# manuelinfosec/corrosion

Hardware: AMD Instinct MI355X
Metric: merged column-changes/sec (node) at 1/2/4/8 GPUs + % of HBM BW roofline (higher is better)
Workload: dtype int64; 1 GPU; config 2: 64M column-changes, 1 table x 4 INTEGER cols, 1000 actors, uniform pk in [1,2^22], cl=1, one apply into an empty state per step; changes=67108864, cells=16469597, parallelism=1 GPU

## Files before the change

corrosion_amd/csrc/engine.hip:

```cpp
#include <hip/hip_runtime.h>

#include <algorithm>
#include <chrono>
#include <cstdlib>
#include <cstring>
#include <mutex>
#include <numeric>

#include "internal.h"
#include "merge_kernels.h"

namespace corro {

static thread_local std::string g_last_error;

void set_error(const std::string &msg) { g_last_error = msg; }

int fail(int code, const std::string &msg) {
    g_last_error = msg;
    return code;
}

int DevBuf::ensure(size_t want) {
    if (want <= bytes && p) return CORRO_OK;
// ... 391 lines not shown
int corro_abi_version(void) { return CORRO_HIP_ABI_VERSION; }

int corro_device_count(int *count) {
    if (!count) return fail(CORRO_E_INVALID, "count is NULL");
    int c = 0;
    hipError_t e = hipGetDeviceCount(&c);
    if (e != hipSuccess) c = 0;
    *count = c;
    return CORRO_OK;
}

static int ctx_prepare_device(corro_ctx *ctx) {
    int c = 0;
    if (hipGetDeviceCount(&c) != hipSuccess || c == 0)
        return fail(CORRO_E_NO_DEVICE, "no HIP device visible: the merge engine has no CPU fallback");
    if (ctx->device < 0 || ctx->device >= c) return fail(CORRO_E_INVALID, "device ordinal out of range");
    CORRO_HIP_TRY(hipSetDevice(ctx->device));
    hipDeviceProp_t prop;
    CORRO_HIP_TRY(hipGetDeviceProperties(&prop, ctx->device));
    if (std::strncmp(prop.gcnArchName, "gfx950", 6) != 0)
        return fail(CORRO_E_NO_DEVICE, std::string("libcorro_hip is built for gfx950, device is ") + prop.gcnArchName);
    CORRO_HIP_TRY(hipStreamCreateWithFlags(&ctx->stream, hipStreamNonBlocking));
    CORRO_HIP_TRY(hipHostMalloc((void **)&ctx->h_misc, MISC_WORDS * sizeof(uint64_t), hipHostMallocDefault));
    for (auto &e : ctx->ev) CORRO_HIP_TRY(hipEventCreate(&e));
    const size_t lds_max = 160 * 1024;
    for (const void *f : {(const void *)k_hist<8>, (const void *)k_hist<16>, (const void *)k_hist<32>,
                          (const void *)k_hist<16, true>, (const void *)k_hist<16, false, true>})
        CORRO_HIP_TRY(hipFuncSetAttribute(f, hipFuncAttributeMaxDynamicSharedMemorySize, (int)lds_max));
    for (const void *f : {(const void *)k_scatter<true, true>, (const void *)k_scatter<true, false>,
                          (const void *)k_scatter<true, false, 8>,
                          (const void *)k_scatter<false, true>, (const void *)k_scatter<false, false>})
        CORRO_HIP_TRY(hipFuncSetAttribute(f, hipFuncAttributeMaxDynamicSharedMemorySize, (int)lds_max));
    return CORRO_OK;
}

}

static int store_alloc(corro_ctx *ctx, uint64_t capacity_hint) {
    const uint32_t B = ctx->B;
    const uint64_t rows = std::max<uint64_t>(1024, capacity_hint / 16);
    uint32_t lg = 4;
    while (((uint64_t)B << lg) < 2 * rows && lg < 20 && ((uint64_t)B << (lg + 1)) <= (1ULL << 31)) lg++;
    ctx->log2S = lg;
    TRY(ctx->d_ent.ensure(((size_t)B << lg) * sizeof(RowEnt)));
    TRY(ctx->d_used.ensure(B * 4ULL));
    TRY(ctx->d_gen.ensure(B * 4ULL));
    TRY(ctx->d_heap_top.ensure(8));
    ctx->heap_cap = std::min<uint64_t>(1ULL << 31, std::max<uint64_t>(1ULL << 16, capacity_hint / 2));
    TRY(ctx->d_heap.ensure(ctx->heap_cap * sizeof(Rec)));
    return CORRO_OK;
}

static int store_clear(corro_ctx *ctx) {
    hipStream_t s = ctx->stream;
    CORRO_HIP_TRY(hipMemsetAsync(ctx->d_ent.p, 0, ((size_t)ctx->B << ctx->log2S) * sizeof(RowEnt), s));
    CORRO_HIP_TRY(hipMemsetAsync(ctx->d_used.p, 0, ctx->B * 4ULL, s));
    CORRO_HIP_TRY(hipMemsetAsync(ctx->d_gen.p, 0, ctx->B * 4ULL, s));
    CORRO_HIP_TRY(hipMemsetAsync(ctx->d_heap_top.p, 0, 8, s));
    if (ctx->d_touch_n.p) CORRO_HIP_TRY(hipMemsetAsync(ctx->d_touch_n.p, 0, 8, s));
    ctx->touch_bound = 0;
    ctx->state_total = 0;
    ctx->state_rows = 0;
    ctx->arena_top = 0;
    ctx->vc_last_bytes = 0;
    ctx->state_epoch++;
    ctx->poisoned = false;
    return CORRO_OK;
}

namespace corro {
RowStore row_store(corro_ctx *ctx) {
    RowStore rs{};
    rs.ent = ctx->d_ent.as<RowEnt>();
    rs.used = ctx->d_used.as<uint32_t>();
    rs.gen = ctx->d_gen.as<uint32_t>();
    rs.heap = ctx->d_heap.as<Rec>();
    rs.heap_ts = ctx->track_ts ? ctx->d_heap_ts.as<uint64_t>() : nullptr;
    rs.heap_top = ctx->d_heap_top.as<unsigned long long>();
    rs.heap_cap = ctx->heap_cap;
    rs.log2S = ctx->log2S;
    rs.fill = (uint32_t)((7ULL << ctx->log2S) >> 3);
    rs.stride = ctx->d_stride.as<uint16_t>();
// ... 98 lines not shown
        }
        Table tb;
        tb.name = tables[t].name;
        for (uint32_t c = 0; c < tables[t].ncols; c++) tb.cols.emplace_back(tables[t].col_names[c]);
        ctx->max_stride = std::max<uint32_t>(ctx->max_stride, tables[t].ncols + 1);
        ctx->table_index[tb.name] = t;
        ctx->tables.push_back(std::move(tb));
    }
    uint64_t per = std::max<uint64_t>(1, capacity_hint / 1280);
    uint32_t lg = 0;
    while ((1ULL << lg) < per && lg < 15) lg++;
    ctx->log2B = lg;
    ctx->B = 1u << lg;
    int rc = ctx_prepare_device(ctx);
    if (rc != CORRO_OK) {
        corro_ctx_destroy(ctx);
        return rc;
    }
    const uint32_t B = ctx->B;
    rc = ctx->d_new_cnt.ensure(B * 4ULL);
    if (!rc) rc = ctx->d_stage_off.ensure(B * 4ULL);
    if (!rc) rc = ctx->d_bflags.ensure(((B + 31) / 32) * 4ULL);
    if (!rc) rc = ctx->d_misc.ensure(MISC_WORDS * 8);
    if (!rc) rc = ctx->d_ovf_list.ensure(B * 4ULL);
    if (!rc) rc = ctx->d_gen_list.ensure(3 * B * 4ULL);
    if (!rc) rc = ctx->d_wide_list.ensure(B * 4ULL);
    if (!rc) rc = ctx->d_defer.ensure(B * 4ULL);
    if (!rc) rc = ctx->d_relist.ensure(B * 4ULL);
    if (!rc) rc = store_alloc(ctx, capacity_hint);
    if (rc != CORRO_OK) {
        corro_ctx_destroy(ctx);
        return rc;
    }
    {
        std::vector<uint16_t> ncols(ctx->tables.size() + 1, 0), stride(ctx->tables.size() + 1, 1);
        for (size_t t = 0; t < ctx->tables.size(); t++) {
            ncols[t] = (uint16_t)ctx->tables[t].cols.size();
            stride[t] = (uint16_t)(ctx->tables[t].cols.size() + 1);
        }
        rc = ctx->d_ncols.ensure(ncols.size() * 2);
        if (!rc) rc = ctx->d_stride.ensure(stride.size() * 2);
        if (rc == CORRO_OK &&
            (hipMemcpy(ctx->d_ncols.p, ncols.data(), ncols.size() * 2, hipMemcpyHostToDevice) != hipSuccess ||
             hipMemcpy(ctx->d_stride.p, stride.data(), stride.size() * 2, hipMemcpyHostToDevice) != hipSuccess))
            rc = fail(CORRO_E_DEVICE, "upload of the schema failed");
        if (rc == CORRO_OK) rc = store_clear(ctx);
        if (rc == CORRO_OK) rc = prims_warm(ctx);
        if (rc == CORRO_OK) rc = agent_dev_reserve(ctx, std::max<uint64_t>(4096, capacity_hint / 64));
        if (rc != CORRO_OK) {
            corro_ctx_destroy(ctx);
            return rc;
        }
    }
    *out = ctx;
    return CORRO_OK;
}

void corro_ctx_destroy(corro_ctx *ctx) {
    if (!ctx) return;
    if (ctx->stream) (void)hipStreamSynchronize(ctx->stream);
    DevBuf *bufs[] = {&ctx->d_site_rank, &ctx->d_dbv, &ctx->d_dbv_batch, &ctx->d_ent, &ctx->d_used, &ctx->d_gen,
                      &ctx->d_heap, &ctx->d_heap_ts, &ctx->d_heap_top, &ctx->d_stride, &ctx->d_defer,
                      &ctx->d_relist, &ctx->d_dense, &ctx->d_dense_ts, &ctx->d_dense_view, &ctx->d_in,
                      &ctx->d_hist, &ctx->d_new_cnt, &ctx->d_stage_off, &ctx->d_bflags, &ctx->d_stage,
                      &ctx->d_misc, &ctx->d_ovf_list, &ctx->d_gen_list, &ctx->d_wide_list, &ctx->d_fast_of, &ctx->d_ovf_sort, &ctx->d_ovf_rcl, &ctx->d_ovf_sum, &ctx->d_ovf_plan, &ctx->d_setdbv,
                      &ctx->d_scan_tmp, &ctx->d_impact, &ctx->d_export, &ctx->d_needs, &ctx->d_needs1,
                      &ctx->d_xidx, &ctx->d_xout, &ctx->d_wire, &ctx->d_wire_schema, &ctx->d_wire_sites,
                      &ctx->d_ncols, &ctx->d_part, &ctx->d_arena, &ctx->d_aff, &ctx->d_affflag,
                      &ctx->d_agent_in, &ctx->d_agent_batch, &ctx->d_agent_spans, &ctx->d_agent_imp,
                      &ctx->d_agent_out, &ctx->d_agent_aux, &ctx->d_agent_fetch, &ctx->d_agent_aux2, &ctx->d_touch, &ctx->d_touch_n, &ctx->d_touch_stamp, &ctx->d_touch_tmp,
                      &ctx->d_aff_conv, &ctx->d_aff_vals, &ctx->d_gaps_big, &ctx->d_agent_hdr, &ctx->d_wire_map,
                      &ctx->d_hdr_stage, &ctx->d_pm_ts};
    for (DevBuf *b : bufs) b->release();
    ctx->d_pkdir.release();
    ctx->d_pk_scratch.release();
    ctx->d_pk_bad.release();
    ctx->d_part_var.release();
    for (PkTable &t : ctx->pk) {
        t.d_off.release();
        t.d_bytes.release();
        t.d_hash.release();
        t.d_slots.release();
    }
    if (ctx->h_misc) (void)hipHostFree(ctx->h_misc);
    if (ctx->h_ovf) (void)hipHostFree(ctx->h_ovf);
    if (ctx->h_agent) (void)hipHostFree(ctx->h_agent);
    if (ctx->h_hdr) (void)hipHostFree(ctx->h_hdr);
    if (ctx->h_hfetch) (void)hipHostFree(ctx->h_hfetch);
// ... 141 lines not shown
static int apply_chunk(corro_ctx *ctx, BatchDev bd, uint8_t *imp_buf) {
    hipStream_t s = ctx->stream;
    const uint32_t n = bd.n;
    const uint32_t B = ctx->B, log2B = ctx->log2B;
    const uint32_t nsites = (uint32_t)ctx->sites.size();
    if (bd.ts && !ctx->track_ts) {
        TRY(ctx->d_heap_ts.ensure(ctx->heap_cap * 8));
        CORRO_HIP_TRY(hipMemsetAsync(ctx->d_heap_ts.p, 0, ctx->heap_cap * 8, s));
        ctx->track_ts = true;
    }

    static const uint32_t tiles_max = [] {
        const char *e = std::getenv("CORRO_HIP_TILES");
        const long v = e ? std::atol(e) : 0;
        return v > 0 && v <= 4096 ? (uint32_t)v : TILES_MAX;
    }();
    uint32_t ntiles = std::max<uint32_t>(1, std::min<uint32_t>(tiles_max, (n + 4095) / 4096));
    uint32_t tile = (n + ntiles - 1) / ntiles;
    tile = (tile + HIST_THREADS - 1) / HIST_THREADS * HIST_THREADS;
    ntiles = (n + tile - 1) / tile;

    TRY(ctx->d_hist.ensure((size_t)ntiles * B * 4));
    TRY(ctx->d_stage.ensure((size_t)n * sizeof(Rec)));
    ApplyZero z{ctx->d_bflags.as<uint32_t>(), ctx->d_misc.as<unsigned long long>(),
                ctx->d_dbv_batch.as<unsigned long long>(), (B + 31) / 32, (uint32_t)MISC_WORDS, nsites};
    if (imp_buf) CORRO_HIP_TRY(hipMemsetAsync(imp_buf, 0, bd.ap ? ctx->pm_n : n, s));

    unsigned long long *misc = ctx->d_misc.as<unsigned long long>();
    const bool prof = ctx->profiling;
    auto mark = [&](int i) {
        if (prof) (void)hipEventRecord(ctx->ev[i], s);
    };
    for (int k = 0; k < 6; k++) ctx->last_ms[k] = 0.f;
    mark(0);
    const uint32_t one_table = ctx->tables.size() == 1 ? 1u : 0u;
    static const int hist_u = std::getenv("CORRO_HIST_U") ? std::atoi(std::getenv("CORRO_HIST_U")) : 16;
    using HistK = void (*)(BatchDev, uint32_t, uint32_t, uint32_t, uint32_t *, ApplyZero);
    const HistK hk = bd.slot_rec ? k_hist<16, true>
                     : !one_table ? (HistK)k_hist<16, false, true>
                     : hist_u == 8 ? k_hist<8> : hist_u == 32 ? k_hist<32> : k_hist<16>;
    hipLaunchKernelGGL(hk, dim3(ntiles), dim3(HIST_THREADS), (size_t)B * 4, s, bd, tile, log2B, one_table,
                       ctx->d_hist.as<uint32_t>(), z);
    CORRO_HIP_TRY(hipGetLastError());
    mark(1);
    hipLaunchKernelGGL(k_colscan, dim3((B + 255) / 256), dim3(256), 0, s, ctx->d_hist.as<uint32_t>(), ntiles, B,
                       ctx->d_new_cnt.as<uint32_t>());
    mark(2);
    hipLaunchKernelGGL(k_plan, dim3(1), dim3(1024), 0, s, ctx->d_new_cnt.as<uint32_t>(), B,
                       ctx->d_stage_off.as<uint32_t>());
    mark(3);
    {
        static const bool nt_stores = std::getenv("CORRO_HIP_NT") && std::atoi(std::getenv("CORRO_HIP_NT")) != 0;
        const bool plain = !bd.v1 && !bd.vt && !bd.vl && !bd.conv;
        if (bd.ts_v1 && !plain) return fail(CORRO_E_INVALID, "internal: ts_v1 on a batch with value words");
        static const bool scat8 = std::getenv("CORRO_SCAT_U") && std::atoi(std::getenv("CORRO_SCAT_U")) == 8;
        auto kern = plain ? (nt_stores ? k_scatter<true, true> : scat8 ? k_scatter<true, false, 8> : k_scatter<true, false>)
                          : (nt_stores ? k_scatter<false, true> : k_scatter<false, false>);
        hipLaunchKernelGGL(kern, dim3(ntiles), dim3(HIST_THREADS), (size_t)B * 4 + ((B + 31) / 32) * 4, s, bd,
                           tile, log2B, one_table, ctx->d_hist.as<uint32_t>(), ctx->d_stage_off.as<uint32_t>(),
                           ctx->d_stage.as<Rec>(), ctx->d_bflags.as<uint32_t>(),
                           ctx->d_dbv_batch.as<unsigned long long>(), nsites, ctx->d_ncols.as<uint16_t>(),
                           (uint32_t)ctx->tables.size(), misc);
    }
    CORRO_HIP_TRY(hipGetLastError());
    mark(4);

    MergeArgs a{};
    a.stage = ctx->d_stage.as<Rec>();
    a.stage_off = ctx->d_stage_off.as<uint32_t>();
    a.new_cnt = ctx->d_new_cnt.as<uint32_t>();
    a.bflags = ctx->d_bflags.as<uint32_t>();
    a.batch_ts = bd.ts;
    a.rs = row_store(ctx);
    a.site_rank = ctx->d_site_rank.as<uint32_t>();
    a.nsites = nsites;
    a.impact = imp_buf;
    a.misc = misc;
    a.ovf_list = ctx->d_ovf_list.as<uint32_t>();
    a.gen_list = ctx->d_gen_list.as<uint32_t>();
    a.wide_list = ctx->d_wide_list.as<uint32_t>();
    a.defer_list = ctx->d_defer.as<uint32_t>();
    a.bucket_list = nullptr;
    a.B = B;
    static const bool force_general = std::getenv("CORRO_HIP_FORCE_GENERAL") &&
                                      std::atoi(std::getenv("CORRO_HIP_FORCE_GENERAL")) != 0;
    a.force_general = force_general ? 1u : 0u;
    static const char *gom = std::getenv("CORRO_GEN_OVF_MIN");
    a.gen_ovf_min = gom ? (uint32_t)std::atoi(gom)
                        : (ovf_reduce_ok(ctx, imp_buf != nullptr) && bd.n >= (1ULL << 24) ? 512u : 0xFFFFFFFFu);
    a.track_ts = ctx->track_ts ? 1u : 0u;
    a.state_wide = ctx->state_wide ? 1u : 0u;
    a.arena = ctx->d_arena.as<uint8_t>();
    a.touch = ctx->track_touched ? ctx->d_touch.as<uint4>() : nullptr;
    a.touch_n = ctx->track_touched ? ctx->d_touch_n.as<unsigned long long>() : nullptr;
    if (bd.conv) {
        a.raw = bd;
        a.raw.arena = ctx->d_arena.as<uint8_t>();
    }
    a.pos_src = bd.ap ? ctx->pm_src : nullptr;
    a.ts_v1 = bd.ts_v1;
    uint32_t nblocks = B;
    float merge_ms = 0.f, ovf_ms = 0.f;
    if (a.impact) {
        CORRO_HIP_TRY(hipMemcpyAsync(ctx->h_misc, misc, (MISC_CVBIG + 1) * 8, hipMemcpyDeviceToHost, s));
        CORRO_HIP_TRY(hipStreamSynchronize(s));
        if (ctx->h_misc[0]) return error_from_bits(ctx->h_misc[0]);
    }
    bool extra_rounds = false;
    for (int round = 0;; round++) {
        if (round > 40) return fail(CORRO_E_NOMEM, "internal: the row store did not take the batch's rows");
        mark(4);
        static const bool no_triage = std::getenv("CORRO_TRIAGE") && std::atoi(std::getenv("CORRO_TRIAGE")) == 0;
        if (!no_triage) {
            TRY(ctx->d_fast_of.ensure(B + 256));
            a.fast_of = ctx->d_fast_of.as<uint8_t>();
            hipLaunchKernelGGL(k_triage, dim3(std::min<uint32_t>((nblocks + 255) / 256, 1024)), dim3(256), 0, s, a, nblocks,
                               ctx->d_fast_of.as<uint8_t>());
            CORRO_HIP_TRY(hipGetLastError());
        }
        if (a.impact) {
            const bool packed = ctx->h_misc[MISC_CVBIG] == 0 && nsites <= 65536;
            auto kern = packed ? k_merge_fast_int<true, true> : k_merge_fast_int<true, false>;
            hipLaunchKernelGGL(kern, dim3(nblocks), dim3(FAST_T), 0, s, a);
            CORRO_HIP_TRY(hipGetLastError());
            hipLaunchKernelGGL(k_merge_fast_wide<true>, dim3(std::min(nblocks, LIST_GRID)), dim3(FAST_T), 0, s, a);
        } else {
            hipLaunchKernelGGL(k_merge_fast_int<false>, dim3(nblocks), dim3(FAST_T), 0, s, a);
            CORRO_HIP_TRY(hipGetLastError());
            hipLaunchKernelGGL(k_merge_fast_wide<false>, dim3(std::min(nblocks, LIST_GRID)), dim3(FAST_T), 0, s, a);
        }
        CORRO_HIP_TRY(hipGetLastError());
        hipLaunchKernelGGL(k_merge_gen_small, dim3(std::min(nblocks, 4 * LIST_GRID)), dim3(GEN_SMALL_THREADS), 0, s, a);
        CORRO_HIP_TRY(hipGetLastError());
        hipLaunchKernelGGL(k_merge_gen_mid, dim3(std::min(nblocks, 2 * LIST_GRID)), dim3(MERGE_THREADS), 0, s, a);
        CORRO_HIP_TRY(hipGetLastError());
        hipLaunchKernelGGL(k_merge_gen, dim3(std::min(nblocks, LIST_GRID)), dim3(MERGE_THREADS), 0, s, a);
        CORRO_HIP_TRY(hipGetLastError());
        mark(5);
        if (round == 0) {
            hipLaunchKernelGGL(k_dbv_fold, dim3((nsites + 255) / 256), dim3(256), 0, s,
                               ctx->d_dbv.as<unsigned long long>(), ctx->d_dbv_batch.as<unsigned long long>(), nsites,
                               (const unsigned long long *)misc);
            CORRO_HIP_TRY(hipMemsetAsync(misc + MISC_ROWS, 0, 8, s));
            hipLaunchKernelGGL(k_sum_used, dim3(1), dim3(1024), 0, s, ctx->d_used.as<uint32_t>(), B, misc);
        }
        CORRO_HIP_TRY(hipMemcpyAsync(ctx->h_misc, misc, MISC_WORDS * 8, hipMemcpyDeviceToHost, s));
        CORRO_HIP_TRY(hipStreamSynchronize(s));
        if (round == 0) {
            if (ctx->h_misc[0]) return error_from_bits(ctx->h_misc[0]);
            ctx->apply_wrote = true;
            if (prof)
                for (int i = 0; i < 4; i++) CORRO_HIP_TRY(hipEventElapsedTime(&ctx->last_ms[i], ctx->ev[i], ctx->ev[i + 1]));
        }
        if (prof) {
            float ms = 0.f;
            CORRO_HIP_TRY(hipEventElapsedTime(&ms, ctx->ev[4], ctx->ev[5]));
            merge_ms += ms;
        }
        const uint64_t novf = ctx->h_misc[MISC_OVF];
        if (novf) {
            extra_rounds = true;
            TRY(run_overflow(ctx, a, novf, n, prof));
            ctx->metrics.overflow_rounds++;
            ovf_ms += ctx->last_ms[5];
        }
        const uint64_t ndefer = ctx->h_misc[MISC_DEFER];
        if (!ndefer) break;
        extra_rounds = true;
        const uint64_t why = ctx->h_misc[MISC_DEFER_WHY];
        ctx->metrics.deferred_rounds++;
        if (why & DEFER_REGION) TRY(grow_regions(ctx, ctx->log2S + 1));
        if (why & DEFER_HEAP) {
            unsigned long long top = 0;
            CORRO_HIP_TRY(hipMemcpy(&top, ctx->d_heap_top.p, 8, hipMemcpyDeviceToHost));
            TRY(grow_heap(ctx, std::max<uint64_t>(ctx->heap_cap * 2, top + (top >> 2))));
        }
        CORRO_HIP_TRY(hipMemcpyAsync(ctx->d_relist.p, ctx->d_defer.p, ndefer * 4, hipMemcpyDeviceToDevice, s));
        for (int w : {MISC_OVF, MISC_GEN, MISC_WIDEQ, MISC_GEN_SMALL, MISC_GEN_MID, MISC_DEFER, MISC_DEFER_WHY})
            CORRO_HIP_TRY(hipMemsetAsync(misc + w, 0, 8, s));
        a.rs = row_store(ctx);
        a.bucket_list = ctx->d_relist.as<uint32_t>();
        nblocks = (uint32_t)ndefer;
    }
    if (prof) {
        ctx->last_ms[4] = merge_ms;
        ctx->last_ms[5] = ovf_ms;
    }
    if (extra_rounds) {
        CORRO_HIP_TRY(hipMemsetAsync(misc + MISC_ROWS, 0, 8, s));
        hipLaunchKernelGGL(k_sum_used, dim3(1), dim3(1024), 0, s, ctx->d_used.as<uint32_t>(), B, misc);
        CORRO_HIP_TRY(hipMemcpyAsync(ctx->h_misc, misc, MISC_WORDS * 8, hipMemcpyDeviceToHost, s));
        CORRO_HIP_TRY(hipStreamSynchronize(s));
    }
    ctx->state_total += ctx->h_misc[MISC_LIVE];
    ctx->state_rows = ctx->h_misc[MISC_ROWS];
#if CORRO_DIAG & 256
    fprintf(stderr, "DIAG impact phases (us per bucket; packed body: loads claims rows counts place walk region winners): %.3f %.3f %.3f %.3f %.3f %.3f %.3f %.3f\n",
            ctx->h_misc[MISC_DIAG] / 100.0 / B, ctx->h_misc[MISC_DIAG + 1] / 100.0 / B,
            ctx->h_misc[MISC_DIAG + 2] / 100.0 / B, ctx->h_misc[MISC_DIAG + 3] / 100.0 / B,
            ctx->h_misc[MISC_DIAG + 4] / 100.0 / B, ctx->h_misc[MISC_DIAG + 5] / 100.0 / B,
            ctx->h_misc[MISC_DIAG + 6] / 100.0 / B, ctx->h_misc[MISC_DIAG + 7] / 100.0 / B);
#endif
#if CORRO_DIAG & 64
    fprintf(stderr, "DIAG phases (us per bucket): load %.3f claims %.3f rows_count %.3f stage1 %.3f stages %.3f fast_rows %.3f winners %.3f publish %.3f\n",
            ctx->h_misc[MISC_DIAG] / 100.0 / B, ctx->h_misc[MISC_DIAG + 1] / 100.0 / B,
            ctx->h_misc[MISC_DIAG + 6] / 100.0 / B, ctx->h_misc[MISC_DIAG + 7] / 100.0 / B,
            ctx->h_misc[MISC_DIAG + 2] / 100.0 / B, ctx->h_misc[MISC_DIAG + 3] / 100.0 / B,
            ctx->h_misc[MISC_DIAG + 4] / 100.0 / B, ctx->h_misc[MISC_DIAG + 5] / 100.0 / B);
#endif
    ctx->state_epoch++;
    if (ctx->h_misc[MISC_WIDE]) ctx->state_wide = true;
    const uint64_t slots = (uint64_t)B << ctx->log2S;
    if (ctx->state_rows * 8 > slots * 5) {
        uint32_t lg = ctx->log2S;
// ... 573 lines not shown
```

corrosion_amd/csrc/internal.h:

```cpp
#pragma once
#include <hip/hip_runtime.h>

#include <array>
#include <cstdint>
#include <cstdlib>
#include <map>
#include <string>
#include <unordered_map>
#include <vector>

#include "corro_hip.h"

namespace corro {

inline bool fault_armed(const char *name) {
    const char *e = std::getenv("CORRO_FAULT");
    if (!e || !*e) return false;
    const std::string s = std::string(",") + e + ",";
    return s.find(std::string(",") + name + ",") != std::string::npos;
}

void set_error(const std::string &msg);
int fail(int code, const std::string &msg);

// ... 131 lines not shown
    const uint64_t *pm_ts = nullptr;
    uint64_t pm_n = 0;
    bool pm_slack = false;
    const void *slot_rec = nullptr;
    const uint64_t *slot_cnt = nullptr;
    uint32_t slot_cap = 0, slot_nsrc = 0;
    uint32_t *slot_over = nullptr;
    bool apply_wrote = false;
    uint64_t heap_limit = 0;
    bool state_wide = false;
    corro::DevBuf d_defer, d_relist;
    corro::DevBuf d_dense, d_dense_ts, d_dense_view;
    corro::DevBuf d_arena;
    uint64_t arena_top = 0;
    uint64_t vc_min_bytes = 0;
    uint64_t vc_last_bytes = 0;
    uint64_t dense_epoch = ~0ULL;

    corro::DevBuf d_in;
    corro::DevBuf d_hist;
    corro::DevBuf d_new_cnt, d_stage_off, d_bflags;
    corro::DevBuf d_stage;
    corro::DevBuf d_misc;
    corro::DevBuf d_ovf_list;
    corro::DevBuf d_gen_list;
    corro::DevBuf d_wide_list;
    corro::DevBuf d_fast_of;
    corro::DevBuf d_ovf_sort;
    corro::DevBuf d_ovf_rcl;
    corro::DevBuf d_ovf_sum;
    bool ovf_sum_dirty = false;
    corro::DevBuf d_ovf_plan;
    uint64_t ovf_temp_k = 0;
    size_t ovf_temp = 0;
    corro::DevBuf d_setdbv;
    corro::DevBuf d_scan_tmp;
    corro::DevBuf d_impact;
    corro::DevBuf d_pm_ts;
    corro::DevBuf d_export;
    corro::DevBuf d_needs;
    corro::DevBuf d_needs1;
    corro::DevBuf d_xidx;
    corro::DevBuf d_xout;
    corro::XIdxPtrs x;
    uint64_t state_epoch = 0;
    uint64_t xidx_epoch = ~0ULL;
// ... 18 lines not shown
    int aff_policy = CORRO_AFF_POLICY_SQLITE_3_37_2;
    corro::DevBuf d_part;
    corro::DevBuf d_pkdir;
    corro::DevBuf d_pk_scratch;
    corro::DevBuf d_pk_bad;
    corro::DevBuf d_part_var;
    corro::DevBuf d_agent_in, d_agent_batch, d_agent_spans, d_agent_imp, d_agent_out, d_agent_aux;
    corro::DevBuf d_agent_fetch, d_agent_aux2;
    corro::DevBuf d_agent_hdr;
    bool agent_sorted_mode = false;
    const uint32_t *agent_src_of = nullptr;
    void *h_agent = nullptr;
    size_t h_agent_bytes = 0;
    void *h_hdr = nullptr;
    size_t h_hdr_bytes = 0;
    void *h_hfetch = nullptr;
    size_t h_hfetch_bytes = 0;
    void *h_pool = nullptr;
    size_t h_pool_bytes = 0;
    corro::DevBuf d_hdr_stage;
    uint64_t agent_ncs = 0;
    uint64_t agent_nbatch_max = 0;
    uint64_t *h_misc = nullptr;
    uint32_t *h_ovf = nullptr;
    bool profiling = false;
    hipEvent_t ev[8] = {};
    float last_ms[9] = {};
};
```

corrosion_amd/csrc/merge_kernels.h:

```cpp
#pragma once
#include "internal.h"
#include "rowhash.h"
#include "rowstore.h"

namespace corro {

#ifndef CORRO_DIAG
#define CORRO_DIAG 0
#endif
constexpr int HIST_THREADS = 512;
constexpr uint64_t CV_PACKED_LIMIT = 1ULL << 15;
constexpr uint32_t TILES_MAX = 256;
constexpr int MERGE_THREADS = 512;
#ifndef CORRO_FAST_T
#define CORRO_FAST_T 512
#endif
constexpr int FAST_T = CORRO_FAST_T;
constexpr int CAP_FAST = 3072;
constexpr int FAST_R = CAP_FAST / FAST_T;
static_assert(FAST_R * FAST_T == CAP_FAST, "FAST_T must divide CAP_FAST");
constexpr int FAST_WAVES_EU = 2 * (FAST_T / 64) / 4;
constexpr int FAST_SLOTS = 4096;
#ifndef IMPACT_LISTS
#define IMPACT_LISTS 0
// ... 112 lines not shown
    w1 = ((in.lbase + off) << 24) | sz;
    return true;
}

__device__ inline void touch_append(const MergeArgs &a, uint64_t pk, uint32_t table) {
    const unsigned long long act = __ballot(1);
    const uint32_t lane = threadIdx.x & 63;
    const uint32_t leader = (uint32_t)__ffsll(act) - 1;
    const uint32_t rank = (uint32_t)__popcll(act & ((1ULL << lane) - 1ULL));
    unsigned long long base = 0;
    if (lane == leader) base = atomicAdd(a.touch_n, (unsigned long long)__popcll(act));
    base = __shfl(base, leader);
    a.touch[base + rank] = make_uint4((uint32_t)pk, (uint32_t)(pk >> 32), table, 0u);
}

__device__ inline uint32_t site_rank_of(const MergeArgs &a, uint32_t site) {
    return site < a.nsites ? a.site_rank[site] : 0u;
}

struct ApplyZero {
    uint32_t *bflags;
    unsigned long long *misc, *dbv_batch;
    uint32_t nbflags, nmisc, nsites;
};
template <int HIST_U, bool SLOT = false, bool MT = false>
static __global__ void __launch_bounds__(HIST_THREADS)
k_hist(BatchDev in, uint32_t tile, uint32_t log2B, uint32_t one_table, uint32_t *__restrict__ hist_out, ApplyZero z) {
    extern __shared__ uint32_t hist[];
    const uint32_t B = 1u << log2B;
    {
        const uint32_t t = blockIdx.x * blockDim.x + threadIdx.x, nt = gridDim.x * blockDim.x;
        for (uint32_t i = t; i < z.nbflags; i += nt) z.bflags[i] = 0;
        for (uint32_t i = t; i < z.nmisc; i += nt) z.misc[i] = 0;
        for (uint32_t i = t; i < z.nsites; i += nt) z.dbv_batch[i] = 0;
    }
    for (uint32_t i = threadIdx.x; i < B; i += blockDim.x) hist[i] = 0;
    bool sover = false;
    if constexpr (SLOT) {
        sover = slot_overflowed(in);
        if (in.slot_over && blockIdx.x == 0 && threadIdx.x == 0) *in.slot_over = sover ? 1u : 0u;
    }
    __syncthreads();
    const uint32_t begin = blockIdx.x * tile;
    const uint32_t end = min(in.n, begin + tile);
    for (uint32_t base = begin; base < end; base += blockDim.x * HIST_U) {
        uint64_t pk[HIST_U];
        uint32_t tc[HIST_U], ap[HIST_U];
#pragma unroll
        for (int k = 0; k < HIST_U; k++) {
            const uint32_t i = min(base + k * blockDim.x + threadIdx.x, end - 1);
            if constexpr (SLOT) {
                pk[k] = in.slot_rec[i].pk;
                tc[k] = one_table ? 0u : in.slot_rec[i].tcid;
                ap[k] = slot_valid(in, i, sover) ? 0u : AP_SKIP;
            } else {
                pk[k] = in.pk[i];
                tc[k] = MT ? in.tcid[i] : 0u;
                ap[k] = in.ap && !in.ap_all ? in.ap[i] : 0u;
            }
        }
#pragma unroll
        for (int k = 0; k < HIST_U; k++) {
            const uint32_t i = base + k * blockDim.x + threadIdx.x;
            if (i < end && ap[k] != AP_SKIP) atomicAdd(&hist[bucket_of(tc[k] >> 16, pk[k], log2B)], 1u);
        }
    }
    __syncthreads();
    uint32_t *row = hist_out + (size_t)blockIdx.x * B;
    for (uint32_t b = threadIdx.x; b < B; b += blockDim.x) row[b] = hist[b];
}

static __global__ void k_colscan(uint32_t *__restrict__ hist, uint32_t ntiles, uint32_t B,
                          uint32_t *__restrict__ new_cnt) {
    const uint32_t b = blockIdx.x * blockDim.x + threadIdx.x;
    if (b >= B) return;
    uint32_t run = 0;
    uint32_t t = 0;
    for (; t + 4 <= ntiles; t += 4) {
        uint32_t c[4];
#pragma unroll
        for (int k = 0; k < 4; k++) c[k] = hist[(size_t)(t + k) * B + b];
#pragma unroll
        for (int k = 0; k < 4; k++) {
            hist[(size_t)(t + k) * B + b] = run;
            run += c[k];
        }
    }
    for (; t < ntiles; t++) {
        const size_t k = (size_t)t * B + b;
        const uint32_t c = hist[k];
        hist[k] = run;
        run += c;
    }
    new_cnt[b] = run;
}

constexpr uint32_t PLAN_PER = 32;
static __global__ void __launch_bounds__(1024)
k_plan(const uint32_t *__restrict__ new_cnt, uint32_t B, uint32_t *__restrict__ stage_off) {
    __shared__ uint64_t w_a[16];
    const uint32_t lane = threadIdx.x & 63, w = threadIdx.x >> 6;
    const uint32_t per = B >= 1024 ? B / 1024 : 1u;
    const uint32_t b0 = threadIdx.x * per;
    const uint32_t cnt = b0 < B ? per : 0u;
    uint64_t sa = 0;
    if (per >= 4) {
        uint4 x[PLAN_PER / 4];
#pragma unroll
        for (uint32_t k = 0; k < PLAN_PER / 4; k++) x[k] = reinterpret_cast<const uint4 *>(new_cnt + b0)[min(k, per / 4 - 1)];
#pragma unroll
        for (uint32_t k = 0; k < PLAN_PER / 4; k++)
            if (4 * k < per) sa += (uint64_t)x[k].x + x[k].y + x[k].z + x[k].w;
    } else {
        for (uint32_t k = 0; k < cnt; k++) sa += new_cnt[b0 + k];
    }
    uint64_t ia = sa;
#pragma unroll
    for (int d = 1; d < 64; d <<= 1) {
        const uint64_t xa = __shfl_up(ia, d);
        if (lane >= (uint32_t)d) ia += xa;
    }
    if (lane == 63) w_a[w] = ia;
    __syncthreads();
    uint64_t ra = ia - sa;
    for (uint32_t ww = 0; ww < w; ww++) ra += w_a[ww];
    if (per >= 4) {
#pragma unroll
        for (uint32_t k = 0; k < PLAN_PER / 4; k++) {
            if (4 * k >= per) break;
            const uint4 xk = reinterpret_cast<const uint4 *>(new_cnt + b0)[k];
            const uint32_t xs[4] = {xk.x, xk.y, xk.z, xk.w};
            uint32_t so[4];
#pragma unroll
            for (int e = 0; e < 4; e++) {
                so[e] = (uint32_t)ra;
                ra += xs[e];
            }
            reinterpret_cast<uint4 *>(stage_off + b0)[k] = make_uint4(so[0], so[1], so[2], so[3]);
        }
    } else {
        for (uint32_t k = 0; k < cnt; k++) {
            stage_off[b0 + k] = (uint32_t)ra;
            ra += new_cnt[b0 + k];
        }
    }
}

__device__ inline void store_rec(Rec *dst, const Rec &r) {
    const uint4 *s = reinterpret_cast<const uint4 *>(&r);
    uint4 *d = reinterpret_cast<uint4 *>(dst);
    d[0] = s[0];
    d[1] = s[1];
    d[2] = s[2];
    d[3] = s[3];
}

__device__ inline Rec load_rec(const Rec *src) {
    Rec r;
    const uint4 *s = reinterpret_cast<const uint4 *>(src);
    uint4 *d = reinterpret_cast<uint4 *>(&r);
    d[0] = s[0];
    d[1] = s[1];
    d[2] = s[2];
    d[3] = s[3];
    return r;
}

__device__ inline void swap32(uint32_t &a, uint32_t &b) {
    auto r = __builtin_amdgcn_permlane32_swap(a, b, false, false);
// ... 2082 lines not shown
        gen_bucket<CAP_GEN, MERGE_THREADS, 0>(a, a.gen_list[k]);
        __syncthreads();
    }
}

static __global__ void __launch_bounds__(MERGE_THREADS, 4)
k_merge_gen_mid(MergeArgs a) {
    const uint32_t cnt = (uint32_t)a.misc[MISC_GEN_MID];
    for (uint32_t k = blockIdx.x; k < cnt; k += gridDim.x) {
        gen_bucket<CAP_GEN_MID, MERGE_THREADS, 2>(a, a.gen_list[2 * a.B + k]);
        __syncthreads();
    }
}

static __global__ void __launch_bounds__(GEN_SMALL_THREADS, 4)
k_merge_gen_small(MergeArgs a) {
    const uint32_t cnt = (uint32_t)a.misc[MISC_GEN_SMALL];
    for (uint32_t k = blockIdx.x; k < cnt; k += gridDim.x) {
        gen_bucket<CAP_GEN_SMALL, GEN_SMALL_THREADS, 1>(a, a.gen_list[a.B + k]);
        __syncthreads();
    }
}

static __global__ void __launch_bounds__(1024) k_sum_used(const uint32_t *__restrict__ used, uint32_t B,
                                                          unsigned long long *misc) {
    unsigned long long t = 0;
    for (uint32_t b = threadIdx.x; b < B; b += 1024) t += used[b];
    for (int d = 32; d >= 1; d >>= 1) t += __shfl_xor(t, d);
    if ((threadIdx.x & 63) == 0 && t) atomicAdd(&misc[MISC_ROWS], t);
}

static __global__ void k_validate(BatchDev in, uint32_t nsites, const uint16_t *__restrict__ ncols, uint32_t ntables,
                                  unsigned long long *misc) {
    uint32_t err = 0, wide = 0;
    const bool sover = in.slot_rec && slot_overflowed(in);
    for (uint32_t i = blockIdx.x * blockDim.x + threadIdx.x; i < in.n; i += gridDim.x * blockDim.x) {
        if (in.slot_rec) {
            if (!slot_valid(in, i, sover)) continue;
            const SlotRec &r = in.slot_rec[i];
            const uint32_t t = r.tcid >> 16, cid = r.tcid & 0xFFFFu;
            if (t >= ntables || cid > ncols[t]) err |= ERR_NAME;
            if (r.site >= nsites) err |= ERR_SITE;
            if ((cid == 0 || (r.cl & 1u) == 0) && (r.cv < 0 || r.cv > 0xFFFFFFFFLL)) err |= ERR_RANGE;
            if (r.dbv < 0) err |= ERR_RANGE;
            continue;
        }
        const uint32_t tc = in.tcid[i], t = tc >> 16, cid = tc & 0xFFFFu, cl = in.cl[i];
        const int64_t cv = in.cv[i];
        if (t >= ntables || cid > ncols[t]) err |= ERR_NAME;
        if (in.site[i] >= nsites) err |= ERR_SITE;
        if ((cid == 0 || (cl & 1u) == 0) && (cv < 0 || cv > 0xFFFFFFFFLL)) err |= ERR_RANGE;
        if (in.dbv[i] < 0) err |= ERR_RANGE;
        if (in.vt) {
            const uint32_t ty = in.vt[i], ln = in.vl ? in.vl[i] : 0u;
            if (ty != CORRO_INTEGER) {
                wide = 1;
                const uint64_t v0 = in.v0[i];
                if (ty < 1 || ty > 5) err |= ERR_VALUE;
                if (ty == CORRO_REAL && ((v0 >> 52) & 0x7FF) == 0x7FF && (v0 & 0xFFFFFFFFFFFFFULL)) err |= ERR_VALUE;
                if ((ty == CORRO_TEXT || ty == CORRO_BLOB) && ln > 16) {
                    uint64_t w0, w1;
                    if (ln != VLEN_LONG || !long_value(in, i, w0, w1)) err |= ERR_VALUE;
                }
            }
        }
    }
    if (__any(err != 0)) {
        for (int d = 32; d >= 1; d >>= 1) err |= __shfl_xor(err, d);
        if ((threadIdx.x & 63) == 0) atomicOr(&misc[0], (unsigned long long)err);
    }
    if (__any(wide != 0) && (threadIdx.x & 63) == 0) atomicOr(&misc[3], 1ULL);
}

static __global__ void k_dbv_fold(unsigned long long *__restrict__ dbv, const unsigned long long *__restrict__ batch,
                           uint32_t nsites, const unsigned long long *__restrict__ misc) {
    const uint32_t i = blockIdx.x * blockDim.x + threadIdx.x;
    if (misc[0]) return;
    if (i < nsites && batch[i] > dbv[i]) dbv[i] = batch[i];
}

template <class F>
__device__ inline void for_each_state_record(const RowStore &rs, uint64_t nent, unsigned long long *count, F &&f) {
    const uint32_t lane = threadIdx.x & 63;
    const uint64_t stride = (uint64_t)gridDim.x * blockDim.x;
    for (uint64_t base = (uint64_t)blockIdx.x * blockDim.x + (threadIdx.x & ~63u); base < nent; base += stride) {
        const uint64_t e = base + lane;
        RowEnt re{};
        if (e < nent) re = rs.ent[e];
        const bool ok = re.tag != 0;
        const uint32_t cnt = ok ? row_popc(re.bits) : 0u;
        uint32_t inc = cnt;
#pragma unroll
        for (int d = 1; d < 64; d <<= 1) {
            const uint32_t y = __shfl_up(inc, d);
            if (lane >= (uint32_t)d) inc += y;
        }
        const uint32_t tot = __shfl(inc, 63);
        unsigned long long w0 = 0;
        if (lane == 63 && tot) w0 = atomicAdd(count, (unsigned long long)tot);
        w0 = __shfl(w0, 63);
        if (!cnt) continue;
// ... 58 lines not shown
}

static __global__ void k_materialize(RowStore rs, uint64_t nent, unsigned long long *count, Rec *out,
                                     uint64_t *out_ts) {
    for_each_state_record(rs, nent, count, [&](unsigned long long k, uint32_t h, int64_t L) {
        Rec r = load_rec(rs.heap + h);
        r.cl = (uint32_t)L;
        r.pos = (uint32_t)k;
        store_rec(out + k, r);
        if (out_ts) out_ts[k] = rs.heap_ts ? rs.heap_ts[h] : 0ULL;
    });
}

static __global__ void k_rehash(const RowEnt *__restrict__ old_ent, uint32_t old_log2S, RowStore rs) {
    const uint32_t b = blockIdx.x;
    const uint32_t S = 1u << old_log2S;
    for (uint32_t s = threadIdx.x; s < S; s += blockDim.x) {
        const RowEnt re = old_ent[((size_t)b << old_log2S) + s];
        if (re.tag == 0) continue;
        rs_insert(rs, b, re.pk, re.tag - 1, re.heap, re.bits);
    }
}

}

#include "ovf_kernels.h"
```

Before: 17.72 billion merged column-changes/s.

## Fuse apply tail launches, decoupled-lookback colscan, and single-kernel store clear

Folds the k_plan exclusive scan into k_colscan using a decoupled lookback across workgroups (atomic ticket ordering plus spin-waits on published totals). The dbv fold, the used-row sum and the misc readback become one tail kernel that writes straight into mapped host memory, replacing a memset, two kernels and a D2H memcpy. Store clear moves from five memsets to one non-temporal clear kernel, and the wide merge kernel is skipped when no wide values are possible. The aim is fewer launches and less serialization on the per-apply critical path, at the cost of spin-wait forward-progress assumptions and relying on zero-copy host-visible writes.

```diff
diff --git a/corrosion_amd/csrc/engine.hip b/corrosion_amd/csrc/engine.hip
--- a/corrosion_amd/csrc/engine.hip
+++ b/corrosion_amd/csrc/engine.hip
@@ -437,6 +437,7 @@
         return fail(CORRO_E_NO_DEVICE, std::string("libcorro_hip is built for gfx950, device is ") + prop.gcnArchName);
     CORRO_HIP_TRY(hipStreamCreateWithFlags(&ctx->stream, hipStreamNonBlocking));
     CORRO_HIP_TRY(hipHostMalloc((void **)&ctx->h_misc, MISC_WORDS * sizeof(uint64_t), hipHostMallocDefault));
+    CORRO_HIP_TRY(hipHostGetDevicePointer((void **)&ctx->h_misc_dev, ctx->h_misc, 0));
     for (auto &e : ctx->ev) CORRO_HIP_TRY(hipEventCreate(&e));
     const size_t lds_max = 160 * 1024;
     for (const void *f : {(const void *)k_hist<8>, (const void *)k_hist<16>, (const void *)k_hist<32>,
@@ -468,11 +469,13 @@
 
 static int store_clear(corro_ctx *ctx) {
     hipStream_t s = ctx->stream;
-    CORRO_HIP_TRY(hipMemsetAsync(ctx->d_ent.p, 0, ((size_t)ctx->B << ctx->log2S) * sizeof(RowEnt), s));
-    CORRO_HIP_TRY(hipMemsetAsync(ctx->d_used.p, 0, ctx->B * 4ULL, s));
-    CORRO_HIP_TRY(hipMemsetAsync(ctx->d_gen.p, 0, ctx->B * 4ULL, s));
-    CORRO_HIP_TRY(hipMemsetAsync(ctx->d_heap_top.p, 0, 8, s));
-    if (ctx->d_touch_n.p) CORRO_HIP_TRY(hipMemsetAsync(ctx->d_touch_n.p, 0, 8, s));
+    const size_t n16 = ((size_t)ctx->B << ctx->log2S) * (sizeof(RowEnt) / 16);
+    static const uint32_t grid_max = std::getenv("CORRO_CLEAR_GRID") ? (uint32_t)std::atoi(std::getenv("CORRO_CLEAR_GRID")) : CLEAR_GRID;
+    static const bool nt = !std::getenv("CORRO_CLEAR_NT") || std::atoi(std::getenv("CORRO_CLEAR_NT")) != 0;
+    const uint32_t grid = (uint32_t)std::min<size_t>(std::max(grid_max, 1u), (n16 + CLEAR_T - 1) / CLEAR_T);
+    hipLaunchKernelGGL(nt ? k_store_clear<true> : k_store_clear<false>, dim3(std::max(grid, 1u)), dim3(CLEAR_T), 0, s,
+                       row_store(ctx), ctx->B, ctx->d_touch_n.as<unsigned long long>());
+    CORRO_HIP_TRY(hipGetLastError());
     ctx->touch_bound = 0;
     ctx->state_total = 0;
     ctx->state_rows = 0;
@@ -617,6 +620,7 @@
     if (!rc) rc = ctx->d_stage_off.ensure(B * 4ULL);
     if (!rc) rc = ctx->d_bflags.ensure(((B + 31) / 32) * 4ULL);
     if (!rc) rc = ctx->d_misc.ensure(MISC_WORDS * 8);
+    if (!rc) rc = ctx->d_colscan.ensure((1 + (B + COLSCAN_T - 1) / COLSCAN_T) * 8ULL);
     if (!rc) rc = ctx->d_ovf_list.ensure(B * 4ULL);
     if (!rc) rc = ctx->d_gen_list.ensure(3 * B * 4ULL);
     if (!rc) rc = ctx->d_wide_list.ensure(B * 4ULL);
@@ -658,7 +662,7 @@
                       &ctx->d_heap, &ctx->d_heap_ts, &ctx->d_heap_top, &ctx->d_stride, &ctx->d_defer,
                       &ctx->d_relist, &ctx->d_dense, &ctx->d_dense_ts, &ctx->d_dense_view, &ctx->d_in,
                       &ctx->d_hist, &ctx->d_new_cnt, &ctx->d_stage_off, &ctx->d_bflags, &ctx->d_stage,
-                      &ctx->d_misc, &ctx->d_ovf_list, &ctx->d_gen_list, &ctx->d_wide_list, &ctx->d_fast_of, &ctx->d_ovf_sort, &ctx->d_ovf_rcl, &ctx->d_ovf_sum, &ctx->d_ovf_plan, &ctx->d_setdbv,
+                      &ctx->d_misc, &ctx->d_colscan, &ctx->d_ovf_list, &ctx->d_gen_list, &ctx->d_wide_list, &ctx->d_fast_of, &ctx->d_ovf_sort, &ctx->d_ovf_rcl, &ctx->d_ovf_sum, &ctx->d_ovf_plan, &ctx->d_setdbv,
                       &ctx->d_scan_tmp, &ctx->d_impact, &ctx->d_export, &ctx->d_needs, &ctx->d_needs1,
                       &ctx->d_xidx, &ctx->d_xout, &ctx->d_wire, &ctx->d_wire_schema, &ctx->d_wire_sites,
                       &ctx->d_ncols, &ctx->d_part, &ctx->d_arena, &ctx->d_aff, &ctx->d_affflag,
@@ -846,8 +850,10 @@
 
     TRY(ctx->d_hist.ensure((size_t)ntiles * B * 4));
     TRY(ctx->d_stage.ensure((size_t)n * sizeof(Rec)));
+    const uint32_t scan_wgs = (B + COLSCAN_T - 1) / COLSCAN_T;
     ApplyZero z{ctx->d_bflags.as<uint32_t>(), ctx->d_misc.as<unsigned long long>(),
-                ctx->d_dbv_batch.as<unsigned long long>(), (B + 31) / 32, (uint32_t)MISC_WORDS, nsites};
+                ctx->d_dbv_batch.as<unsigned long long>(), (B + 31) / 32, (uint32_t)MISC_WORDS, nsites,
+                ctx->d_colscan.as<unsigned long long>(), 1 + scan_wgs};
     if (imp_buf) CORRO_HIP_TRY(hipMemsetAsync(imp_buf, 0, bd.ap ? ctx->pm_n : n, s));
 
     unsigned long long *misc = ctx->d_misc.as<unsigned long long>();
@@ -867,15 +873,13 @@
                        ctx->d_hist.as<uint32_t>(), z);
     CORRO_HIP_TRY(hipGetLastError());
     mark(1);
-    hipLaunchKernelGGL(k_colscan, dim3((B + 255) / 256), dim3(256), 0, s, ctx->d_hist.as<uint32_t>(), ntiles, B,
-                       ctx->d_new_cnt.as<uint32_t>());
+    hipLaunchKernelGGL(k_colscan, dim3(scan_wgs), dim3(COLSCAN_T), 0, s, ctx->d_hist.as<uint32_t>(), ntiles, B,
+                       ctx->d_new_cnt.as<uint32_t>(), ctx->d_stage_off.as<uint32_t>(),
+                       ctx->d_colscan.as<unsigned long long>());
     mark(2);
-    hipLaunchKernelGGL(k_plan, dim3(1), dim3(1024), 0, s, ctx->d_new_cnt.as<uint32_t>(), B,
-                       ctx->d_stage_off.as<uint32_t>());
-    mark(3);
+    const bool plain = !bd.v1 && !bd.vt && !bd.vl && !bd.conv;
     {
         static const bool nt_stores = std::getenv("CORRO_HIP_NT") && std::atoi(std::getenv("CORRO_HIP_NT")) != 0;
-        const bool plain = !bd.v1 && !bd.vt && !bd.vl && !bd.conv;
         if (bd.ts_v1 && !plain) return fail(CORRO_E_INVALID, "internal: ts_v1 on a batch with value words");
         static const bool scat8 = std::getenv("CORRO_SCAT_U") && std::atoi(std::getenv("CORRO_SCAT_U")) == 8;
         auto kern = plain ? (nt_stores ? k_scatter<true, true> : scat8 ? k_scatter<true, false, 8> : k_scatter<true, false>)
@@ -887,7 +891,7 @@
                            (uint32_t)ctx->tables.size(), misc);
     }
     CORRO_HIP_TRY(hipGetLastError());
-    mark(4);
+    mark(3);
 
     MergeArgs a{};
     a.stage = ctx->d_stage.as<Rec>();
@@ -931,9 +935,10 @@
         if (ctx->h_misc[0]) return error_from_bits(ctx->h_misc[0]);
     }
     bool extra_rounds = false;
+    const bool wide_possible = ctx->state_wide || !plain;
     for (int round = 0;; round++) {
         if (round > 40) return fail(CORRO_E_NOMEM, "internal: the row store did not take the batch's rows");
-        mark(4);
+        if (round > 0 || a.impact) mark(4);
         static const bool no_triage = std::getenv("CORRO_TRIAGE") && std::atoi(std::getenv("CORRO_TRIAGE")) == 0;
         if (!no_triage) {
             TRY(ctx->d_fast_of.ensure(B + 256));
@@ -947,11 +952,13 @@
             auto kern = packed ? k_merge_fast_int<true, true> : k_merge_fast_int<true, false>;
             hipLaunchKernelGGL(kern, dim3(nblocks), dim3(FAST_T), 0, s, a);
             CORRO_HIP_TRY(hipGetLastError());
-            hipLaunchKernelGGL(k_merge_fast_wide<true>, dim3(std::min(nblocks, LIST_GRID)), dim3(FAST_T), 0, s, a);
+            if (wide_possible)
+                hipLaunchKernelGGL(k_merge_fast_wide<true>, dim3(std::min(nblocks, LIST_GRID)), dim3(FAST_T), 0, s, a);
         } else {
             hipLaunchKernelGGL(k_merge_fast_int<false>, dim3(nblocks), dim3(FAST_T), 0, s, a);
             CORRO_HIP_TRY(hipGetLastError());
-            hipLaunchKernelGGL(k_merge_fast_wide<false>, dim3(std::min(nblocks, LIST_GRID)), dim3(FAST_T), 0, s, a);
+            if (wide_possible)
+                hipLaunchKernelGGL(k_merge_fast_wide<false>, dim3(std::min(nblocks, LIST_GRID)), dim3(FAST_T), 0, s, a);
         }
         CORRO_HIP_TRY(hipGetLastError());
         hipLaunchKernelGGL(k_merge_gen_small, dim3(std::min(nblocks, 4 * LIST_GRID)), dim3(GEN_SMALL_THREADS), 0, s, a);
@@ -962,23 +969,24 @@
         CORRO_HIP_TRY(hipGetLastError());
         mark(5);
         if (round == 0) {
-            hipLaunchKernelGGL(k_dbv_fold, dim3((nsites + 255) / 256), dim3(256), 0, s,
-                               ctx->d_dbv.as<unsigned long long>(), ctx->d_dbv_batch.as<unsigned long long>(), nsites,
-                               (const unsigned long long *)misc);
-            CORRO_HIP_TRY(hipMemsetAsync(misc + MISC_ROWS, 0, 8, s));
-            hipLaunchKernelGGL(k_sum_used, dim3(1), dim3(1024), 0, s, ctx->d_used.as<uint32_t>(), B, misc);
-        }
-        CORRO_HIP_TRY(hipMemcpyAsync(ctx->h_misc, misc, MISC_WORDS * 8, hipMemcpyDeviceToHost, s));
+            hipLaunchKernelGGL(k_apply_tail, dim3(1), dim3(TAIL_T), 0, s, ctx->d_dbv.as<unsigned long long>(),
+                               ctx->d_dbv_batch.as<unsigned long long>(), nsites, ctx->d_used.as<uint32_t>(), B, misc,
+                               ctx->h_misc_dev);
+            CORRO_HIP_TRY(hipGetLastError());
+        } else {
+            CORRO_HIP_TRY(hipMemcpyAsync(ctx->h_misc, misc, MISC_WORDS * 8, hipMemcpyDeviceToHost, s));
+        }
         CORRO_HIP_TRY(hipStreamSynchronize(s));
         if (round == 0) {
             if (ctx->h_misc[0]) return error_from_bits(ctx->h_misc[0]);
             ctx->apply_wrote = true;
             if (prof)
-                for (int i = 0; i < 4; i++) CORRO_HIP_TRY(hipEventElapsedTime(&ctx->last_ms[i], ctx->ev[i], ctx->ev[i + 1]));
+                for (int i = 0; i < 3; i++)
+                    CORRO_HIP_TRY(hipEventElapsedTime(&ctx->last_ms[i == 2 ? 3 : i], ctx->ev[i], ctx->ev[i + 1]));
         }
         if (prof) {
             float ms = 0.f;
-            CORRO_HIP_TRY(hipEventElapsedTime(&ms, ctx->ev[4], ctx->ev[5]));
+            CORRO_HIP_TRY(hipEventElapsedTime(&ms, ctx->ev[round > 0 || a.impact ? 4 : 3], ctx->ev[5]));
             merge_ms += ms;
         }
         const uint64_t novf = ctx->h_misc[MISC_OVF];
@@ -1011,9 +1019,10 @@
         ctx->last_ms[5] = ovf_ms;
     }
     if (extra_rounds) {
-        CORRO_HIP_TRY(hipMemsetAsync(misc + MISC_ROWS, 0, 8, s));
-        hipLaunchKernelGGL(k_sum_used, dim3(1), dim3(1024), 0, s, ctx->d_used.as<uint32_t>(), B, misc);
-        CORRO_HIP_TRY(hipMemcpyAsync(ctx->h_misc, misc, MISC_WORDS * 8, hipMemcpyDeviceToHost, s));
+        hipLaunchKernelGGL(k_apply_tail, dim3(1), dim3(TAIL_T), 0, s, ctx->d_dbv.as<unsigned long long>(),
+                           ctx->d_dbv_batch.as<unsigned long long>(), 0u, ctx->d_used.as<uint32_t>(), B, misc,
+                           ctx->h_misc_dev);
+        CORRO_HIP_TRY(hipGetLastError());
         CORRO_HIP_TRY(hipStreamSynchronize(s));
     }
     ctx->state_total += ctx->h_misc[MISC_LIVE];
diff --git a/corrosion_amd/csrc/internal.h b/corrosion_amd/csrc/internal.h
--- a/corrosion_amd/csrc/internal.h
+++ b/corrosion_amd/csrc/internal.h
@@ -177,6 +177,7 @@
     corro::DevBuf d_new_cnt, d_stage_off, d_bflags;
     corro::DevBuf d_stage;
     corro::DevBuf d_misc;
+    corro::DevBuf d_colscan;
     corro::DevBuf d_ovf_list;
     corro::DevBuf d_gen_list;
     corro::DevBuf d_wide_list;
@@ -241,6 +242,7 @@
     uint64_t agent_ncs = 0;
     uint64_t agent_nbatch_max = 0;
     uint64_t *h_misc = nullptr;
+    unsigned long long *h_misc_dev = nullptr;
     uint32_t *h_ovf = nullptr;
     bool profiling = false;
     hipEvent_t ev[8] = {};
diff --git a/corrosion_amd/csrc/merge_kernels.h b/corrosion_amd/csrc/merge_kernels.h
--- a/corrosion_amd/csrc/merge_kernels.h
+++ b/corrosion_amd/csrc/merge_kernels.h
@@ -158,6 +158,8 @@
     uint32_t *bflags;
     unsigned long long *misc, *dbv_batch;
     uint32_t nbflags, nmisc, nsites;
+    unsigned long long *scan;
+    uint32_t nscan;
 };
 template <int HIST_U, bool SLOT = false, bool MT = false>
 static __global__ void __launch_bounds__(HIST_THREADS)
@@ -169,6 +171,7 @@
         for (uint32_t i = t; i < z.nbflags; i += nt) z.bflags[i] = 0;
         for (uint32_t i = t; i < z.nmisc; i += nt) z.misc[i] = 0;
         for (uint32_t i = t; i < z.nsites; i += nt) z.dbv_batch[i] = 0;
+        for (uint32_t i = t; i < z.nscan; i += nt) z.scan[i] = 0;
     }
     for (uint32_t i = threadIdx.x; i < B; i += blockDim.x) hist[i] = 0;
     bool sover = false;
@@ -206,81 +209,70 @@
     for (uint32_t b = threadIdx.x; b < B; b += blockDim.x) row[b] = hist[b];
 }
 
-static __global__ void k_colscan(uint32_t *__restrict__ hist, uint32_t ntiles, uint32_t B,
-                          uint32_t *__restrict__ new_cnt) {
-    const uint32_t b = blockIdx.x * blockDim.x + threadIdx.x;
-    if (b >= B) return;
+constexpr uint32_t COLSCAN_T = 256;
+constexpr unsigned long long COLSCAN_DONE = 1ULL << 63;
+static __global__ void __launch_bounds__(COLSCAN_T)
+k_colscan(uint32_t *__restrict__ hist, uint32_t ntiles, uint32_t B, uint32_t *__restrict__ new_cnt,
+          uint32_t *__restrict__ stage_off, unsigned long long *scan) {
+    __shared__ uint32_t s_wg, s_w[COLSCAN_T / 64];
+    __shared__ unsigned long long s_base;
+    if (threadIdx.x == 0) s_wg = (uint32_t)atomicAdd(&scan[0], 1ULL);
+    __syncthreads();
+    const uint32_t wg = s_wg;
+    const uint32_t lane = threadIdx.x & 63, w = threadIdx.x >> 6;
+    const uint32_t b = wg * COLSCAN_T + threadIdx.x;
     uint32_t run = 0;
-    uint32_t t = 0;
-    for (; t + 4 <= ntiles; t += 4) {
-        uint32_t c[4];
-#pragma unroll
-        for (int k = 0; k < 4; k++) c[k] = hist[(size_t)(t + k) * B + b];
-#pragma unroll
-        for (int k = 0; k < 4; k++) {
-            hist[(size_t)(t + k) * B + b] = run;
-            run += c[k];
-        }
-    }
-    for (; t < ntiles; t++) {
-        const size_t k = (size_t)t * B + b;
-        const uint32_t c = hist[k];
-        hist[k] = run;
-        run += c;
-    }
-    new_cnt[b] = run;
+    if (b < B) {
+        uint32_t t = 0;
+        for (; t + 4 <= ntiles; t += 4) {
+            uint32_t c[4];
+#pragma unroll
+            for (int k = 0; k < 4; k++) c[k] = hist[(size_t)(t + k) * B + b];
+#pragma unroll
+            for (int k = 0; k < 4; k++) {
+                hist[(size_t)(t + k) * B + b] = run;
+                run += c[k];
+            }
+        }
+        for (; t < ntiles; t++) {
+            const size_t k = (size_t)t * B + b;
+            const uint32_t c = hist[k];
+            hist[k] = run;
+            run += c;
+        }
+        new_cnt[b] = run;
+    }
+    uint32_t incl = run;
+#pragma unroll
+    for (int d = 1; d < 64; d <<= 1) {
+        const uint32_t x = __shfl_up(incl, d);
+        if (lane >= (uint32_t)d) incl += x;
+    }
+    if (lane == 63) s_w[w] = incl;
+    __syncthreads();
+    uint32_t before = incl - run, total = 0;
+    for (uint32_t ww = 0; ww < COLSCAN_T / 64; ww++) {
+        if (ww < w) before += s_w[ww];
+        total += s_w[ww];
+    }
+    if (threadIdx.x == 0)
+        __hip_atomic_store(&scan[1 + wg], COLSCAN_DONE | total, __ATOMIC_RELAXED, __HIP_MEMORY_SCOPE_AGENT);
+    if (w == 0) {
+        unsigned long long sum = 0;
+        for (uint32_t j = lane; j < wg; j += 64) {
+            unsigned long long st;
+            while (!((st = __hip_atomic_load(&scan[1 + j], __ATOMIC_RELAXED, __HIP_MEMORY_SCOPE_AGENT)) & COLSCAN_DONE))
+                __builtin_amdgcn_s_sleep(1);
+            sum += st & ~COLSCAN_DONE;
+        }
+        for (int d = 32; d >= 1; d >>= 1) sum += __shfl_xor(sum, d);
+        if (lane == 0) s_base = sum;
+    }
+    __syncthreads();
+    if (b < B) stage_off[b] = (uint32_t)s_base + before;
 }
 
 constexpr uint32_t PLAN_PER = 32;
-static __global__ void __launch_bounds__(1024)
-k_plan(const uint32_t *__restrict__ new_cnt, uint32_t B, uint32_t *__restrict__ stage_off) {
-    __shared__ uint64_t w_a[16];
-    const uint32_t lane = threadIdx.x & 63, w = threadIdx.x >> 6;
-    const uint32_t per = B >= 1024 ? B / 1024 : 1u;
-    const uint32_t b0 = threadIdx.x * per;
-    const uint32_t cnt = b0 < B ? per : 0u;
-    uint64_t sa = 0;
-    if (per >= 4) {
-        uint4 x[PLAN_PER / 4];
-#pragma unroll
-        for (uint32_t k = 0; k < PLAN_PER / 4; k++) x[k] = reinterpret_cast<const uint4 *>(new_cnt + b0)[min(k, per / 4 - 1)];
-#pragma unroll
-        for (uint32_t k = 0; k < PLAN_PER / 4; k++)
-            if (4 * k < per) sa += (uint64_t)x[k].x + x[k].y + x[k].z + x[k].w;
-    } else {
-        for (uint32_t k = 0; k < cnt; k++) sa += new_cnt[b0 + k];
-    }
-    uint64_t ia = sa;
-#pragma unroll
-    for (int d = 1; d < 64; d <<= 1) {
-        const uint64_t xa = __shfl_up(ia, d);
-        if (lane >= (uint32_t)d) ia += xa;
-    }
-    if (lane == 63) w_a[w] = ia;
-    __syncthreads();
-    uint64_t ra = ia - sa;
-    for (uint32_t ww = 0; ww < w; ww++) ra += w_a[ww];
-    if (per >= 4) {
-#pragma unroll
-        for (uint32_t k = 0; k < PLAN_PER / 4; k++) {
-            if (4 * k >= per) break;
-            const uint4 xk = reinterpret_cast<const uint4 *>(new_cnt + b0)[k];
-            const uint32_t xs[4] = {xk.x, xk.y, xk.z, xk.w};
-            uint32_t so[4];
-#pragma unroll
-            for (int e = 0; e < 4; e++) {
-                so[e] = (uint32_t)ra;
-                ra += xs[e];
-            }
-            reinterpret_cast<uint4 *>(stage_off + b0)[k] = make_uint4(so[0], so[1], so[2], so[3]);
-        }
-    } else {
-        for (uint32_t k = 0; k < cnt; k++) {
-            stage_off[b0 + k] = (uint32_t)ra;
-            ra += new_cnt[b0 + k];
-        }
-    }
-}
 
 __device__ inline void store_rec(Rec *dst, const Rec &r) {
     const uint4 *s = reinterpret_cast<const uint4 *>(&r);
@@ -2409,14 +2401,6 @@
     }
 }
 
-static __global__ void __launch_bounds__(1024) k_sum_used(const uint32_t *__restrict__ used, uint32_t B,
-                                                          unsigned long long *misc) {
-    unsigned long long t = 0;
-    for (uint32_t b = threadIdx.x; b < B; b += 1024) t += used[b];
-    for (int d = 32; d >= 1; d >>= 1) t += __shfl_xor(t, d);
-    if ((threadIdx.x & 63) == 0 && t) atomicAdd(&misc[MISC_ROWS], t);
-}
-
 static __global__ void k_validate(BatchDev in, uint32_t nsites, const uint16_t *__restrict__ ncols, uint32_t ntables,
                                   unsigned long long *misc) {
     uint32_t err = 0, wide = 0;
@@ -2459,11 +2443,39 @@
     if (__any(wide != 0) && (threadIdx.x & 63) == 0) atomicOr(&misc[3], 1ULL);
 }
 
-static __global__ void k_dbv_fold(unsigned long long *__restrict__ dbv, const unsigned long long *__restrict__ batch,
-                           uint32_t nsites, const unsigned long long *__restrict__ misc) {
-    const uint32_t i = blockIdx.x * blockDim.x + threadIdx.x;
-    if (misc[0]) return;
-    if (i < nsites && batch[i] > dbv[i]) dbv[i] = batch[i];
+constexpr uint32_t TAIL_T = 1024;
+static __global__ void __launch_bounds__(TAIL_T)
+k_apply_tail(unsigned long long *__restrict__ dbv, const unsigned long long *__restrict__ batch, uint32_t nsites,
+             const uint32_t *__restrict__ used, uint32_t B, unsigned long long *misc, unsigned long long *out) {
+    __shared__ unsigned long long s_w[TAIL_T / 64];
+    unsigned long long t = 0;
+    if (B >= 4) {
+        const uint32_t n4 = B / 4;
+        uint4 x[PLAN_PER / 4];
+#pragma unroll
+        for (uint32_t k = 0; k < PLAN_PER / 4; k++)
+            x[k] = reinterpret_cast<const uint4 *>(used)[min(threadIdx.x + k * TAIL_T, n4 - 1)];
+#pragma unroll
+        for (uint32_t k = 0; k < PLAN_PER / 4; k++)
+            if (threadIdx.x + k * TAIL_T < n4) t += (unsigned long long)x[k].x + x[k].y + x[k].z + x[k].w;
+    } else if (threadIdx.x < B) {
+        t = used[threadIdx.x];
+    }
+    for (int d = 32; d >= 1; d >>= 1) t += __shfl_xor(t, d);
+    if ((threadIdx.x & 63) == 0) s_w[threadIdx.x >> 6] = t;
+    if (!misc[0])
+        for (uint32_t i = threadIdx.x; i < nsites; i += TAIL_T)
+            if (batch[i] > dbv[i]) dbv[i] = batch[i];
+    __syncthreads();
+    if (threadIdx.x < (uint32_t)MISC_WORDS) {
+        unsigned long long v = misc[threadIdx.x];
+        if (threadIdx.x == (uint32_t)MISC_ROWS) {
+            v = 0;
+            for (uint32_t ww = 0; ww < TAIL_T / 64; ww++) v += s_w[ww];
+            misc[MISC_ROWS] = v;
+        }
+        out[threadIdx.x] = v;
+    }
 }
 
 template <class F>
@@ -2568,6 +2580,34 @@
     }
 }
 
+constexpr uint32_t CLEAR_T = 256, CLEAR_GRID = 256;
+template <bool NT>
+static __global__ void __launch_bounds__(CLEAR_T)
+k_store_clear(RowStore rs, uint32_t B, unsigned long long *touch_n) {
+    const uint32_t t = blockIdx.x * CLEAR_T + threadIdx.x, nt = gridDim.x * CLEAR_T;
+    uint4 *ent = reinterpret_cast<uint4 *>(rs.ent);
+    const size_t n16 = ((size_t)B << rs.log2S) * (sizeof(RowEnt) / 16);
+    const uint4 zero = make_uint4(0u, 0u, 0u, 0u);
+#pragma unroll 4
+    for (size_t i = t; i < n16; i += nt) {
+        if (NT) {
+            typedef uint32_t v4u __attribute__((ext_vector_type(4)));
+            const v4u z = {0u, 0u, 0u, 0u};
+            __builtin_nontemporal_store(z, reinterpret_cast<v4u *>(ent + i));
+        } else {
+            ent[i] = zero;
+        }
+    }
+    for (uint32_t b = t; b < B; b += nt) {
+        rs.used[b] = 0;
+        rs.gen[b] = 0;
+    }
+    if (t == 0) {
+        *rs.heap_top = 0;
+        if (touch_n) *touch_n = 0;
+    }
+}
+
 }
 
 #include "ovf_kernels.h"
```

Result: faster. 18.04 billion merged column-changes/s, median of 6 (+1.8%).
